# k2-fsa/Flow2GAN

Measured on AMD Instinct MI355X. Metric: audio-seconds/sec (train step, G+D fwd/bwd) mel_24k_base, higher is better.
Workload: dtype f32 (fp32-class products on the bf16 matrix pipe for the long reductions and the direct MRD convs: every fp32 operand as three bf16 pieces = 24 significand bits, the six v_mfma_f32_32x32x16_bf16 products with i + j <= 2 per fp32 product, fp32 accumulate, error <= 2^-23 per product; short reductions ; 1 GPU; mel_24k_base GAN stage-2 train step: D-step + G-step, each on its own batch (MPD+MRD+FM+multi-scale mel), fwd+bwd+grad all-reduce, no optimizer (metric is fwd/bwd); per_gpu_batch=64, gan=gan_multi_scale_mel_recon, parallelism=dp1, optimizer=none

## Files before the change

flow2gan_amd/_lib.py:

```python
from __future__ import annotations

import ctypes as C
import os

import torch

_HERE = os.path.dirname(os.path.abspath(__file__))
LIB_PATH = os.environ.get("F2G_LIB_PATH") or os.path.join(_HERE, "libflow2gan_hip.so")

c_float_p = C.c_void_p


class Operand(C.Structure):
    _fields_ = [
        ("base", C.c_void_p), ("rows", C.c_int32), ("cols", C.c_int32),
        ("P1", C.c_int32), ("P0", C.c_int32), ("seglen", C.c_int32),
        ("step1", C.c_int32), ("pad1", C.c_int32), ("L1", C.c_int32),
        ("step0", C.c_int32), ("pad0", C.c_int32), ("unit", C.c_int32), ("L0u", C.c_int32),
        ("seq_stride", C.c_int64), ("line_stride", C.c_int64),
        ("reflect", C.c_int32), ("split", C.c_int32),
        ("alpha", C.c_void_p), ("lrelu_src", C.c_void_p),
        ("lrelu_slope", C.c_float), ("unbounded", C.c_int32),
        ("rscale", C.c_void_p),
    ]
# ... 195 lines not shown
    "f2g_wave_gain": [_P, _L, _P, _L, _L, _I, _I, _I, _P, _P, _P],
    "f2g_sadam_stats": [_P, _P, _I, _P, _I],
    "f2g_sadam_prepare": [_P, C.POINTER(SadamGroup), _P, _P, _P, _P],
    "f2g_lrelu_bwd_colsum": [_P, _P, _P, _F, _P, _F, _I, _I, _L, _P],
    "f2g_lrelu_bwd_add": [_P, _P, _L, _I, _I, _I, _I, _L, _L, _L, _P, _L, _L, _L, _L, _F, _P],
    "f2g_zero_halo": [_P, _I, _I, _I, _I, _I],
    "f2g_sadam_update": [_P, _P, _I, _P],
    "f2g_mlp_pack": [_P, _P, _L, _P, _L, _I, _I],
    "f2g_fused_mlp": [C.POINTER(FusedMlpDesc)],
    "f2g_fused_block": [C.POINTER(DwnormFwd), C.POINTER(FusedMlpDesc)],
    "f2g_fused_block_multi": [C.POINTER(DwnormFwd), C.POINTER(FusedMlpDesc), C.c_int32],
    "f2g_istft_ola_multi": [C.POINTER(OlaMultiDesc), _P, _I, _I, _F, _I],
    "f2g_split_bf16x3": [_P, _P, _L, _I, _I],
    "f2g_split_f16x2": [_P, _P, _P, _L, _I, _I],
    "f2g_split_f16x2_cols": [_P, _P, _P, _P, _L, _I, _I],
    "f2g_split_f16x2_seq": [_P, _P, _P, _L, _I, _I],
    "f2g_multi": [C.POINTER(MultiDesc)],
}
EXPORTS = sorted(list(_SIGS) + ["f2g_version", "f2g_last_error", "f2g_gemm_last_path", "f2g_gemm_last_kernel",
                                 "f2g_fused_last_launch", "f2g_convnext_last_launch",
                                 "f2g_gemm_lean_ok", "f2g_gemm_wgrad_lean", "f2g_fused_mlp_ok",
                                 "f2g_dwnorm_bwd_workspace", "f2g_split_bf16x3_bytes", "f2g_gemm_x6_ok",
                                 "f2g_gemm_colsum_part_rows", "f2g_gemm_f16_ok", "f2g_set_option", "f2g_get_option",
                                 "f2g_dwconv_bwd_workspace", "f2g_sadam_chunk_elems"])


class F2GError(RuntimeError):
    pass


def _load():
    if not os.path.exists(LIB_PATH):
        raise ImportError(
            f"{LIB_PATH} is missing: build it with `python -c 'import __graft_entry__ as g; "
            "g.build()'` (or `make -C flow2gan_amd/csrc`). There is no CPU fallback.")
    lib = C.CDLL(LIB_PATH)
    for name, args in _SIGS.items():
        fn = getattr(lib, name)
        fn.argtypes = list(args) + [C.c_void_p]
        fn.restype = C.c_int
    for name in ("f2g_dwnorm_bwd_workspace", "f2g_dwconv_bwd_workspace"):
        fn = getattr(lib, name)
        fn.argtypes = [C.c_int32] * 4
        fn.restype = C.c_int64
    lib.f2g_gemm_lean_ok.argtypes = [C.POINTER(GemmDesc)]
    lib.f2g_gemm_lean_ok.restype = C.c_int
    lib.f2g_gemm_wgrad_lean.argtypes = [C.POINTER(GemmDesc)]
    lib.f2g_gemm_wgrad_lean.restype = C.c_int
    lib.f2g_split_bf16x3_bytes.argtypes = [C.c_int32, C.c_int32]
    lib.f2g_split_bf16x3_bytes.restype = C.c_int64
    lib.f2g_gemm_x6_ok.argtypes = [C.POINTER(GemmDesc)]
    lib.f2g_gemm_x6_ok.restype = C.c_int
    lib.f2g_gemm_f16_ok.argtypes = [C.POINTER(GemmDesc)]
    lib.f2g_gemm_f16_ok.restype = C.c_int
    lib.f2g_gemm_colsum_part_rows.argtypes = [C.POINTER(GemmDesc)]
    lib.f2g_gemm_colsum_part_rows.restype = C.c_int32
    lib.f2g_fused_mlp_ok.argtypes = [C.c_int32, C.c_int32]
    lib.f2g_fused_mlp_ok.restype = C.c_int
    lib.f2g_sadam_chunk_elems.argtypes = []
    lib.f2g_sadam_chunk_elems.restype = C.c_int32
    lib.f2g_set_option.argtypes = [C.c_char_p, C.c_int32]
    lib.f2g_set_option.restype = C.c_int
    lib.f2g_get_option.argtypes = [C.c_char_p, C.POINTER(C.c_int32)]
    lib.f2g_get_option.restype = C.c_int
    lib.f2g_version.restype = C.c_char_p
    lib.f2g_last_error.restype = C.c_char_p
    lib.f2g_gemm_last_kernel.argtypes = []
    lib.f2g_gemm_last_kernel.restype = C.c_char_p
    lib.f2g_fused_last_launch.argtypes = []
# ... 61 lines not shown
```

flow2gan_amd/csrc/capi.hip:

```cpp
#include <stdio.h>
#include <stdlib.h>
#include <string.h>
#include <strings.h>

#include <mutex>

#include "common.h"
#include "version_gen.h"

static char g_err[256] = "";

void f2g_set_error(const char* msg) {
  strncpy(g_err, msg ? msg : "", sizeof(g_err) - 1);
  g_err[sizeof(g_err) - 1] = 0;
}

int f2g_check_launch() {
  hipError_t e = hipGetLastError();
  if (e != hipSuccess) {
    f2g_set_error(hipGetErrorString(e));
    return F2G_ELAUNCH;
  }
  return F2G_OK;
}

extern "C" const char* f2g_version(void) { return "flow2gan_hip 0.4.0 src:" F2G_SRC_HASH " gfx950"; }
extern "C" const char* f2g_last_error(void) { return g_err; }

namespace {
struct Opt { const char* name; int value; };
Opt g_opts[F2G_OPT_COUNT] = {
    {"lean_tall", 1}, {"lean_wgrad", 1}, {"x6p", 1}, {"deterministic", 0}, {"streamk", 1}, {"mlp_rt", 0},
    {"mlp_split", 0}, {"multi_rt384", 4}, {"multi_rt512", 3}, {"streamk_min", 4}};
std::once_flag g_opts_once;

int opt_index(const char* name, size_t len) {
  for (int i = 0; i < F2G_OPT_COUNT; ++i)
    if (strlen(g_opts[i].name) == len && strncasecmp(g_opts[i].name, name, len) == 0) return i;
  return -1;
}

void opts_init() {
  const char* e = getenv("F2G_OPTS");
  while (e && *e) {
    const char* end = strchr(e, ',');
    const size_t len = end ? (size_t)(end - e) : strlen(e);
    const char* eq = (const char*)memchr(e, '=', len);
    if (eq) {
      const int i = opt_index(e, (size_t)(eq - e));
      if (i >= 0) g_opts[i].value = atoi(eq + 1);
    }
    e = end ? end + 1 : nullptr;
  }
  const char* det = getenv("F2G_DETERMINISTIC");
  if (det) g_opts[F2G_OPT_DETERMINISTIC].value = atoi(det) != 0;
}
// ... 26 lines not shown
```

flow2gan_amd/csrc/common.h:

```cpp
#pragma once
#include <hip/hip_runtime.h>
#include <stdint.h>

#include <type_traits>

#include "../../include/flow2gan_hip.h"

int f2g_check_launch();
void f2g_note_kernel(const char* name, int split, int path);
enum f2g_opt_id {
  F2G_OPT_LEAN_TALL,
  F2G_OPT_LEAN_WGRAD,
  F2G_OPT_X6P,
  F2G_OPT_DETERMINISTIC,
  F2G_OPT_STREAMK,
  F2G_OPT_MLP_RT,
  F2G_OPT_MLP_SPLIT,
  F2G_OPT_MULTI_RT384,
  F2G_OPT_MULTI_RT512,
  F2G_OPT_STREAMK_MIN,
  F2G_OPT_COUNT
};
int f2g_opt(int id);
int f2g_gemm_narrow(const f2g_gemm_desc& d, hipStream_t st);
void f2g_set_error(const char* msg);
int f2g_x6p_ok(const f2g_gemm_desc& d, int taps);
int f2g_launch_x6p(const f2g_gemm_desc& d, int taps, long long a_extent, hipStream_t st);
int f2g_leanw6t_ok(const f2g_gemm_desc& d, int split);
int f2g_launch_leanw6t(const f2g_gemm_desc& d, int split, hipStream_t st);
struct f2g_colsegs {
  float* out[3];
  int begin[3];
  int count[3];
};
int f2g_colsum_segments(const float* a, long long lda, int rows, int ncols,
                        const f2g_colsegs& segs, hipStream_t st);

#define F2G_WAVE 64

__device__ __forceinline__ float wave_sum(float v) {
#pragma unroll
  for (int o = 32; o > 0; o >>= 1) v += __shfl_xor(v, o);
  return v;
}

__device__ __forceinline__ float wave_max(float v) {
#pragma unroll
  for (int o = 32; o > 0; o >>= 1) v = fmaxf(v, __shfl_xor(v, o));
  return v;
}

typedef float f2g_f32x2 __attribute__((ext_vector_type(2)));
// ... 27 lines not shown
```

flow2gan_amd/csrc/gemm.hip:

```cpp
#include <hip/hip_runtime.h>
#include <stddef.h>
#include <stdint.h>
#include <stdio.h>
#include <string.h>

#include "gemm_common.h"

namespace {

int g_last_path = 0;
const char* g_last_kernel = "";
int g_last_split = 1;

struct RowCtx {
  long long base;
  int l1b, e0;
};

__device__ __forceinline__ RowCtx decode_row(const f2g_operand& S, int r) {
  RowCtx rc;
  int s, p1, p0;
  if (S.P0 == 1 && S.P1 == 1) {
    s = r; p1 = 0; p0 = 0;
  } else {
// ... 737 lines not shown
  hipLaunchKernelGGL(split_bf16_kernel, dim3((unsigned)blocks), dim3(256), 0, (hipStream_t)stream,
                     reinterpret_cast<uint4*>(dst), reinterpret_cast<const float4*>(src), n4);
  return f2g_check_launch();
}

extern "C" int f2g_gemm(const f2g_gemm_desc* dp, f2g_stream_t stream) {
  if (!dp || !dp->A.base || !dp->B.base || !dp->E.C) return F2G_EINVAL;
  f2g_note_kernel("", 1, g_last_path);
  const f2g_gemm_desc& d = *dp;
  hipStream_t st = (hipStream_t)stream;
  int split = d.split_k > 0 ? d.split_k : 1;
  if (d.E.colsum_part_ld > 0 && f2g_gemm_colsum_part_rows(dp) == 0) {
    f2g_set_error("f2g_gemm: E.colsum_part_ld needs a launch with the wide epilogue "
                  "(f2g_gemm_colsum_part_rows(d) == 0 for this descriptor)");
    return F2G_EINVAL;
  }
  if (d.precision == 4) return f2g_gemm_h3(d, st);
  if ((d.A.split >= 5 && d.A.split <= 8) || (d.B.split >= 5 && d.B.split <= 8)) {
    f2g_set_error("f2g_gemm: f2g_split_f16x2 / _cols / _seq images (split = 5 / 6 / 7) and maps scaled inside the "
                  "kernel (split = 8) belong to precision 4");
    return F2G_EINVAL;
  }
  if (d.precision == 3 && d.form == 2) {
    if (d.A.split || d.B.split || d.A.rows != d.B.rows || !f2g_leanw_ok(d) || d.E.x3_out ||
        (split > 1 && !d.E.atomic)) {
      f2g_set_error("f2g_gemm precision 3, form 2: fp32 operands the K-major weight-gradient kernel reads");
      return F2G_EINVAL;
    }
    return f2g_launch_leanw(d, 6, split, st);
  }
  if (d.precision == 3) return f2g_gemm_x6(d, st);
  if (d.E.x3_out) {
    f2g_set_error("f2g_gemm: E.x3_out belongs to precision 3");
    return F2G_EINVAL;
  }
  {
    const int nr = f2g_gemm_narrow(d, st);
    if (nr != 0) return nr < 0 ? nr : F2G_OK;
    f2g_note_kernel("", 1, 0);
  }
  if (d.E.prelu_slope && (d.E.atomic || d.E.accumulate || d.E.P0o > 0 || d.form == 2)) return F2G_EINVAL;
  if (d.E.mask_src && (d.E.atomic || d.E.accumulate || d.form == 2)) return F2G_EINVAL;
  if (d.form == 0 || d.form == 1) {
    const bool f1 = d.form == 1;
    if (f1 ? d.A.cols != d.B.rows : d.A.cols != d.B.cols) return F2G_EINVAL;
    if (!host_plain(d.B)) return F2G_EINVAL;
// ... 64 lines not shown
```

flow2gan_amd/csrc/gemm_x6.hip:

```cpp
#include <stddef.h>
#include <stdint.h>

#include "gemm_common.h"
#include "x6_epilogue.h"

#define X6_MFMA_PRIO 1

#if F2G_X6LAB & 256
__device__ unsigned long long g_x6prof[8];
extern "C" int f2g_lab_x6prof(unsigned long long* out8) {
  unsigned long long z[8] = {0, 0, 0, 0, 0, 0, 0, 0};
  if (hipMemcpyFromSymbol(out8, HIP_SYMBOL(g_x6prof), sizeof(z)) != hipSuccess) return 1;
  return hipMemcpyToSymbol(HIP_SYMBOL(g_x6prof), z, sizeof(z)) != hipSuccess;
}
#endif

__global__ __launch_bounds__(256) void split3_img_kernel(__bf16* __restrict__ dst, const float* __restrict__ src,
                                                         long long ld, long long rows, int K) {
  const long long total = rows * (K / 4);
  for (long long i = (long long)blockIdx.x * blockDim.x + threadIdx.x; i < total;
       i += (long long)gridDim.x * blockDim.x) {
    const long long r = i / (K / 4);
    const int k4 = (int)(i - r * (K / 4)) * 4;
    const float4 v = *reinterpret_cast<const float4*>(src + r * ld + k4);
// ... 599 lines not shown
  if (d.E.x3_out) {
    const f2g_epilogue& E = d.E;
    if (E.prelu_out || (((uintptr_t)E.x3_out) & 15) || (((uintptr_t)E.C) & 15) || (N % 8)) return false;
    if (E.P0o > 0 ? ((E.seq_stride_o | E.row_stride_o | E.off_o) & 7) != 0 : (E.ldc & 7) != 0) return false;
  }
  return true;
}

static int x6_wide(const f2g_gemm_desc& d) {
  return x6e::wide_ok(d.E, d.B.rows) ? 1 : 0;
}

static bool x6f_ok(const f2g_gemm_desc& d) {
  if (d.A.split || (d.B.split != 0 && d.B.split != 3 && d.B.split != 4) || !x6_shape_ok(d)) return false;
  if (d.B.split == 4 && ((d.B.rows & 31) || d.B.rows <= 32 || d.B.P0 != 1 || d.B.P1 != 1)) return false;
  if (!al16(d.A.base) || !al16(d.B.base) || (d.A.seq_stride & 3) || (d.B.split == 0 && (d.B.seq_stride & 3))) return false;
  const long long ext = host_plain(d.A) ? (long long)d.A.rows * d.A.seq_stride : x6_a_extent(d.A);
  return ext * 4 < 0xe0000000ll && (long long)d.B.rows * (d.B.split ? d.B.cols * 6ll : d.B.seq_stride * 4) < 0xe0000000ll;
}

enum x6_kind {
  X6_NONE,
  X6_P,
  X6_IMG,
  X6_F,
  X6_G,
  X6_N
};
struct x6_pick {
  x6_kind kind;
  int arg;
};

static x6_pick x6_choose(const f2g_gemm_desc& d) {
  if (x6f_ok(d)) {
    if (d.B.rows <= 32 && d.B.split == 3 && !d.E.x3_out) return {X6_N, 0};
    if (d.B.split == 4) return {X6_G, 0};
    return {X6_F, d.B.split == 3 ? 1 : 0};
  }
  if (d.A.split != 3 || d.B.split != 3 || !x6_shape_ok(d)) return {X6_NONE, 0};
  for (int taps = 5; taps >= 2; taps -= 3)
    if (x6_tap_ok(d, taps) && f2g_x6p_ok(d, taps)) return {X6_P, taps};
  return {X6_IMG, 0};
}

static x6_rows x6_rows_of(const f2g_operand& A, int es) {
  x6_rows R;
  if (host_plain(A)) {
    const long long pitch = es == 6 ? A.cols : A.seq_stride;
    R.P0 = 1, R.seq6 = (unsigned)(pitch * es), R.step6 = 0, R.off6 = 0;
    R.bytes = (unsigned)((long long)A.rows * pitch * es);
  } else {
    R.P0 = A.P0, R.seq6 = (unsigned)(A.seq_stride * es);
    R.step6 = (unsigned)((long long)A.step0 * A.unit * es), R.off6 = (unsigned)(-(long long)A.pad0 * A.unit * es);
    R.bytes = (unsigned)(x6_a_extent(A) * es);
  }
  return R;
}

int f2g_gemm_x6(const f2g_gemm_desc& d, hipStream_t st) {
  const int M = d.A.rows, N = d.B.rows, K = d.A.cols;
  constexpr size_t smem = 2 * 128 * 208;
  const dim3 grid((M + 127) / 128, (N + 127) / 128);
  const x6_pick pick = x6_choose(d);
  switch (pick.kind) {
    case X6_NONE:
      f2g_set_error("f2g_gemm precision 3: form 0 over plain f2g_split_bf16x3 images (split = 3), K % 32 == 0");
      return F2G_EINVAL;
    case X6_P:
      return f2g_launch_x6p(d, pick.arg, x6_a_extent(d.A), st);
    case X6_IMG:
      dyn_lds_once<gemm_x6_kernel>((int)smem);
      f2g_note_kernel("x6", 1, 4);
      hipLaunchKernelGGL(gemm_x6_kernel, grid, dim3(256), smem, st, d, M, N, K, x6_rows_of(d.A, 6), x6_wide(d));
      break;
    case X6_N: {
      constexpr size_t smem_n = (128 + 32) * 208;
      f2g_note_kernel("x6n", 1, 5);
      hipLaunchKernelGGL(gemm_x6n_kernel, dim3((M + 127) / 128), dim3(256), smem_n, st, d, M, N, K, x6_rows_of(d.A, 4));
      break;
    }
    case X6_G: {
      constexpr size_t smem_g = 4 * x6e::ESZ > 128 * 208 ? 4 * x6e::ESZ : 128 * 208;
      f2g_note_kernel("x6g", 1, 4);
      hipLaunchKernelGGL(gemm_x6g_kernel, grid, dim3(256), smem_g, st, d, M, N, K, x6_rows_of(d.A, 4), x6_wide(d));
      break;
    }
    case X6_F:
      dyn_lds_once<gemm_x6f_kernel<false>, gemm_x6f_kernel<true>>((int)smem);
      f2g_note_kernel(pick.arg ? "x6f<wimg=1>" : "x6f<wimg=0>", 1, 4);
      hipLaunchKernelGGL(pick.arg ? gemm_x6f_kernel<true> : gemm_x6f_kernel<false>, grid, dim3(256), smem, st, d, M, N,
                         K, x6_rows_of(d.A, 4), x6_wide(d));
      break;
  }
  return f2g_check_launch();
}

extern "C" int f2g_gemm_x6_ok(const f2g_gemm_desc* d) {
  if (!d || !x6_shape_ok(*d)) return 0;
  return 1 | ((x6_tap_ok(*d, 5) || x6_tap_ok(*d, 2)) ? 2 : 0) | (x6f_ok(*d) ? 4 : 0);
}

extern "C" int32_t f2g_gemm_colsum_part_rows(const f2g_gemm_desc* dp) {
  if (!dp || (dp->precision != 3 && dp->precision != 4) || dp->form != 0) return 0;
  f2g_gemm_desc d = *dp;
  if (d.E.colsum_part_ld <= 0) d.E.colsum_part_ld = 4;
  if (d.precision == 4 && d.A.split == 8) return f2g_h3p3n_ok(d) ? 2 * ((d.A.rows + 127) / 128) : 0;
  if (d.precision == 4) return f2g_h3p_ok(d, nullptr) || f2g_h3p3_ok(d) ? 4 * ((d.A.rows + 255) / 256) : 0;
  if (!x6_wide(d)) return 0;
  const int M = d.A.rows;
  switch (x6_choose(d).kind) {
    case X6_NONE:
    case X6_N:
      return 0;
    case X6_P:
      return 4 * ((M + 255) / 256);
    default:
      return 2 * ((M + 127) / 128);
  }
}

extern "C" int64_t f2g_split_bf16x3_bytes(int32_t rows, int32_t K) { return (int64_t)rows * K * 6; }

extern "C" int f2g_split_bf16x3(void* dst, const float* src, int64_t ld, int32_t rows, int32_t K,
                                f2g_stream_t stream) {
  if (!dst || !src || rows < 0 || K < 32 || (K % 32) || ld < K || (ld & 3) || (((uintptr_t)src) & 15) ||
      (((uintptr_t)dst) & 15))
    return F2G_EINVAL;
  if (rows == 0) return F2G_OK;
  const long long total = (long long)rows * (K / 4);
  hipLaunchKernelGGL(split3_img_kernel, dim3(f2g_grid_for(total, 256)), dim3(256), 0, (hipStream_t)stream,
                     reinterpret_cast<__bf16*>(dst), src, (long long)ld, (long long)rows, K);
  return f2g_check_launch();
}
```

flow2gan_amd/csrc/gemm_x6p.hip:

```cpp
#include <stdlib.h>

#include "gemm_common.h"
#include "x6_epilogue.h"

namespace {

constexpr int PITCH = 208;
constexpr int LH = 160;
constexpr int OPERA = 2 * LH * PITCH;
constexpr int OPERB = 128 * PITCH;
using x6e::ESZ;

struct x6p_tap {
  int P0, HpIn, offpos, C32;
  unsigned bytes;
};

template <int TAPS>
__global__ __launch_bounds__(512, 1) void gemm_x6p_kernel(const f2g_gemm_desc d, int M, int N, int K,
                                                          const x6p_tap R) {
  extern __shared__ __attribute__((aligned(16))) unsigned char smem6[];
  constexpr int NJA = (LH * 12 + 255) / 256, NJB = 128 * 12 / 512;
  const int tid = threadIdx.x, lane = tid & 63, wave = tid >> 6;
  const int grp = wave >> 2, gt = tid & 255;
// ... 89 lines not shown
            fb[ks][p][i] = *reinterpret_cast<const bf16x8*>(rB + buf * OPERB + p * 64 + i * 32 * PITCH + ks * 32);
          }
      storeB(buf ^ 1);
      gloadB(slab_of(step + 2));
      lds_barrier();
      if (t == TAPS - 1 && cs + 1 < R.C32) {
        storeA();
        gloadA(cs + 2 < R.C32 ? cs + 2 : 0);
      }
      __builtin_amdgcn_s_setprio(1);
#pragma unroll
      for (int ks = 0; ks < 2; ++ks)
#pragma unroll
        for (int sdeg = 2; sdeg >= 0; --sdeg)
#pragma unroll
          for (int i = 0; i < 3; ++i) {
            const int j = sdeg - i;
            if (j < 0 || j > 2) continue;
#pragma unroll
            for (int mi = 0; mi < 2; ++mi)
#pragma unroll
              for (int ni = 0; ni < 2; ++ni)
                acc[mi][ni] = __builtin_amdgcn_mfma_f32_32x32x16_bf16(fa[ks][i][mi], fb[ks][j][ni], acc[mi][ni], 0, 0, 0);
          }
      __builtin_amdgcn_s_setprio(0);
      if (!(grp == 1 && step == nsteps - 1)) lds_barrier();
    }
  }
  x6e::wide_epilogue(d.E, acc, M, N, mg + wm * 64, n0 + wn * 64, lane, smem6 + wave * ESZ);
}



template <int TAPS>
__global__ __launch_bounds__(512, 1) void gemm_leanw6t_kernel(const f2g_gemm_desc d, int K, int kchunk,
                                                              long long xrows) {
  constexpr int XR = 32 + TAPS - 1;
  constexpr int GPL = 32 * 256, XPL = XR * 256;
  constexpr int BUFB = 3 * GPL + 3 * XPL;
  constexpr int NXQ = (XR * 32 + 511) / 512;
  extern __shared__ __attribute__((aligned(16))) unsigned char smw[];
  const int tid = threadIdx.x, lane = tid & 63, wave = tid >> 6;
  const int wm = wave & 1, wq = wave >> 1, li = lane & 31, h = lane >> 5;
  const int m0 = blockIdx.x * 128, c0 = blockIdx.y * 128;
  const int kbeg = blockIdx.z * kchunk;
  int kend = kbeg + kchunk;
// ... 253 lines not shown
  const int mode = f2g_opt(F2G_OPT_X6P);
  if (mode == 0 || (taps != 5 && taps != 2)) return 0;
  if (d.A.unit / 32 < 2) return 0;
  if (!x6e::wide_ok(d.E, d.B.rows)) return 0;
  const long long tiles = (long long)((d.A.rows + 255) / 256) * ((d.B.rows + 127) / 128);
  return (mode >= 2 || tiles >= 256) ? 1 : 0;
}

int f2g_launch_x6p(const f2g_gemm_desc& d, int taps, long long a_extent, hipStream_t st) {
  const int M = d.A.rows, N = d.B.rows, K = d.A.cols;
  constexpr size_t smem = (size_t)OPERA + 2 * OPERB;
  static_assert(8 * ESZ <= (int)smem, "epilogue patches fit under the main loop's buffers");
  dyn_lds_once<gemm_x6p_kernel<5>, gemm_x6p_kernel<2>>((int)smem);
  x6p_tap R;
  R.P0 = d.A.P0, R.HpIn = (int)(d.A.seq_stride / d.A.unit), R.offpos = -d.A.pad0, R.C32 = d.A.unit / 32;
  R.bytes = (unsigned)(a_extent * 6);
  dim3 grid((M + 255) / 256, (N + 127) / 128);
  f2g_note_kernel(taps == 5 ? "x6p<taps=5>" : "x6p<taps=2>", 1, 4);
  if (taps == 5) hipLaunchKernelGGL(gemm_x6p_kernel<5>, grid, dim3(512), smem, st, d, M, N, K, R);
  else hipLaunchKernelGGL(gemm_x6p_kernel<2>, grid, dim3(512), smem, st, d, M, N, K, R);
  return f2g_check_launch();
}

int f2g_leanw6t_ok(const f2g_gemm_desc& d, int split) {
  const f2g_operand& A = d.A;
  const f2g_operand& B = d.B;
  if (d.form != 2 || d.precision != 3 || !d.E.atomic || d.E.P0o > 0 || d.E.bias || d.E.res) return 0;
  const f2g_epilogue& E = d.E;
  if ((E.scale != 0.f && E.scale != 1.f) || E.colsum || E.colsum_alpha || E.lrelu_slope != 0.f || E.mask_src ||
      E.aux || E.prelu_slope || E.c_bf16 || E.x3_out || E.accumulate || A.lrelu_src || A.alpha || B.lrelu_src || B.alpha)
    return 0;
  if (B.P1 != 1 || B.P0 < 1 || (B.step0 != 1 && B.step0 != 3) || B.unit < 128 || (B.unit % 128) || !B.unbounded) return 0;
  if (B.cols != 5 * B.unit || B.seglen < B.cols || (B.seq_stride % B.unit) || (B.rows % B.P0)) return 0;
  if (A.cols % 128 || A.rows != B.rows || B.pad0 < 0 || B.pad0 > 8) return 0;
  if (B.step0 == 1 && B.seq_stride != (long long)B.P0 * B.unit) return 0;
  const long long xrows = (long long)(B.rows / B.P0) * (B.seq_stride / B.unit);
  if (xrows * B.unit * 4 >= 0x7ff00000ll || (long long)A.rows * A.seq_stride * 4 >= 0x7ff00000ll) return 0;
  return 1;
}

int f2g_launch_leanw6t(const f2g_gemm_desc& d, int split, hipStream_t st) {
  const int M = d.A.cols, K = d.A.rows, Cin = d.B.unit;
  constexpr int TAPS = 5;
  if (d.B.step0 == 3) {
    constexpr size_t smem3 = (size_t)2 * (3 * 16 * 256 + 3 * (15 * 3 + TAPS) * 256);
    dyn_lds_once<gemm_leanw6s_kernel<5, 3>>((int)smem3);
// ... 41 lines not shown
```

flow2gan_amd/ops.py:

```python
from __future__ import annotations

import ctypes as C
from typing import Optional

import torch

from . import _lib as L
from ._opts import opt
from ._lib import DwconvBwd, DwnormBwd, DwnormFwd, Epilogue, GemmDesc, Operand, call, ptr


def empty(*shape, device, dtype=torch.float32):
    return torch.empty(*shape, device=device, dtype=dtype)


def zeros(*shape, device):
    t = torch.empty(*shape, device=device, dtype=torch.float32)
    fill_(t, 0.0)
    return t


def fill_(t, v: float):
    if BATCH is not None and t.numel() > 0:
        import struct
# ... 430 lines not shown
        if X6F == 2 and 128 <= A.cols < X6_MIN_K and A.rows >= X6F_TALL_ROWS and Bm.rows == 32:
            in_kernel = True
        if X6F == 2 and X6_MIN_K <= A.cols < X6_NOPASS_K and A.P0 == 1 and A.P1 == 1 and not _is_const(A._keep[0]):
            in_kernel = True
        if form == 0 and A.split == 0 and Bm.split == 0 and A.rows >= X6_MIN_ROWS \
                and (A.cols >= X6_MIN_K or in_kernel) and not atomic \
                and split_k <= 1 and out.dtype == torch.float32 and _x3_window_ok(A):
            how = _ask_with_x3_out(d, out, out_offset, x3_out, prelu_out, lambda: L.lib.f2g_gemm_x6_ok(C.byref(d)))
            if how:
                if in_kernel and not (how & 4):
                    in_kernel = False
                    how = how if A.cols >= X6_MIN_K else 0
                if how:
                    if not in_kernel:
                        d.A, d.B = _x3_operand(A), _x3_operand(Bm)
                    elif Bm.P0 == 1 and Bm.P1 == 1 and _is_const(Bm._keep[0]):
                        d.B = _x3_operand(Bm, frag_major=X6G and Bm.rows % 32 == 0 and Bm.rows > 32)
                    d.precision = 3
            if d.precision != 3:
                d.E.x3_out = None
        if form == 2 and atomic and A.split == 0 and Bm.split == 0 and A.lrelu_src is None \
                and A.rows >= X6_MIN_K and L.lib.f2g_gemm_lean_ok(C.byref(d)):
            d.precision = 3
        if x3_out:
            if d.E.x3_out:
                out._f2g_x3 = out._f2g_x3_buf
            else:
                out._f2g_x3_bad = True
    if (GEMM_PRECISION == 1 and form in (0, 2)) or (GEMM_PRECISION == 2 and form == 0):
        ok = L.lib.f2g_gemm_lean_ok(C.byref(d))
        if GEMM_PRECISION == 2 and (ok & 2):
            d.A, d.B = _bf16_operand(A), _bf16_operand(Bm)
        elif ok:
            d.A, d.B = _split_operand(A), _split_operand(Bm)
    parts = None
    if COLSUM_PARTS and d.precision in (3, 4) and form == 0 and (colsum is not None or colsum_alpha is not None) \
            and A.rows >= COLSUM_PARTS_MIN_ROWS:
        nrows = L.lib.f2g_gemm_colsum_part_rows(C.byref(d))
        if nrows > 0:
            ncol = Bm.rows
            both = colsum is not None and colsum_alpha is not None
            parts = torch.empty(nrows, (2 if both else 1) * ncol, device=out.device, dtype=torch.float32)
            d.E.colsum_part_ld = parts.stride(0)
            if colsum_alpha is not None:
                d.E.colsum_alpha = ptr(parts)
            if colsum is not None:
# ... 1406 lines not shown
```

include/flow2gan_hip.h:

```cpp
#ifndef FLOW2GAN_HIP_H
#define FLOW2GAN_HIP_H

#include <stdint.h>

#ifdef __cplusplus
extern "C" {
#endif

typedef void* f2g_stream_t;

enum {
  F2G_OK = 0,
  F2G_EINVAL = -1,
  F2G_ELAUNCH = -2,
};

const char* f2g_version(void);
const char* f2g_last_error(void);

int f2g_set_option(const char* name, int32_t value);
int f2g_get_option(const char* name, int32_t* value);

typedef struct {
  const float* base;
// ... 35 lines not shown
  float* prelu_out;
  int64_t ld_prelu_out;
  const float* mask_src;
  const float* fm_ref;
  const float* fm_wdev;
  float mask_slope;
  float fm_w;
  void* x3_out;
  int64_t colsum_part_ld;
} f2g_epilogue;

typedef struct {
  f2g_operand A, B;
  f2g_epilogue E;
  int32_t form;
  int32_t split_k;
  int32_t precision;
  int32_t _pad3;
} f2g_gemm_desc;

int f2g_gemm(const f2g_gemm_desc* d, f2g_stream_t stream);
int f2g_gemm_wgrad_lean(const f2g_gemm_desc* d);
int f2g_gemm_lean_ok(const f2g_gemm_desc* d);
int f2g_split_bf16(float* dst, const float* src, int64_t n, f2g_stream_t stream);
int f2g_to_bf16(void* dst, const float* src, int64_t n, f2g_stream_t stream);
int64_t f2g_split_bf16x3_bytes(int32_t rows, int32_t K);
int f2g_split_bf16x3(void* dst, const float* src, int64_t ld, int32_t rows, int32_t K, f2g_stream_t stream);
int f2g_gemm_x6_ok(const f2g_gemm_desc* d);
int32_t f2g_gemm_colsum_part_rows(const f2g_gemm_desc* d);
int f2g_split_f16x2(float* dst, float* rscale, const float* src, int64_t ld, int32_t rows, int32_t K,
                    f2g_stream_t stream);
int f2g_gemm_f16_ok(const f2g_gemm_desc* d);
int f2g_split_f16x2_cols(float* dst, float* rscale, uint32_t* work, const float* src, int64_t ld, int32_t rows,
                         int32_t cols, f2g_stream_t stream);
int f2g_split_f16x2_seq(float* dst, float* rscale, const float* src, int64_t ld, int32_t nseq, int32_t seq_floats,
                        f2g_stream_t stream);

int f2g_gemm_last_path(void);
const char* f2g_gemm_last_kernel(void);

typedef struct {
  const float* x;
  int64_t ldx;
  float* z;
  int64_t ldz;
  int32_t B, F, C, K;
// ... 326 lines not shown
```

Baseline: 810.8 audio-s/s.

## Add specialized bf16x3 kernels for stride-3 five-tap conv forward and weight gradient

Adds two new MFMA kernels specialized for the stride-3, 5-tap conv pattern used in the MPD discriminator. The first, x6p3, is a forward kernel that stages each input plane once in LDS and reuses it across taps in an interleaved tap order. The second, leanw6n, is a weight-gradient kernel that splits fp32 into three bf16 planes while staging and reads them with transposed LDS loads, then accumulates taps atomically. Both come with new eligibility checks and option flags, and the Python dispatcher now routes matching weight-gradient GEMMs to leanw6n. The aim is to cut the im2col-style operand traffic and split passes for these convs, at the cost of more code paths and atomic-add nondeterminism.

Measured after the change: 816.6 audio-s/s, median of 6. No clear change (+0.7%).

```diff
diff --git a/flow2gan_amd/_lib.py b/flow2gan_amd/_lib.py
--- a/flow2gan_amd/_lib.py
+++ b/flow2gan_amd/_lib.py
@@ -241,7 +241,7 @@
                                  "f2g_gemm_lean_ok", "f2g_gemm_wgrad_lean", "f2g_fused_mlp_ok",
                                  "f2g_dwnorm_bwd_workspace", "f2g_split_bf16x3_bytes", "f2g_gemm_x6_ok",
                                  "f2g_gemm_colsum_part_rows", "f2g_gemm_f16_ok", "f2g_set_option", "f2g_get_option",
-                                 "f2g_dwconv_bwd_workspace", "f2g_sadam_chunk_elems"])
+                                 "f2g_dwconv_bwd_workspace", "f2g_sadam_chunk_elems", "f2g_leanw6n_ok"])
 
 
 class F2GError(RuntimeError):
@@ -264,6 +264,8 @@
         fn.restype = C.c_int64
     lib.f2g_gemm_lean_ok.argtypes = [C.POINTER(GemmDesc)]
     lib.f2g_gemm_lean_ok.restype = C.c_int
+    lib.f2g_leanw6n_ok.argtypes = [C.POINTER(GemmDesc)]
+    lib.f2g_leanw6n_ok.restype = C.c_int
     lib.f2g_gemm_wgrad_lean.argtypes = [C.POINTER(GemmDesc)]
     lib.f2g_gemm_wgrad_lean.restype = C.c_int
     lib.f2g_split_bf16x3_bytes.argtypes = [C.c_int32, C.c_int32]
diff --git a/flow2gan_amd/csrc/capi.hip b/flow2gan_amd/csrc/capi.hip
--- a/flow2gan_amd/csrc/capi.hip
+++ b/flow2gan_amd/csrc/capi.hip
@@ -31,7 +31,7 @@
 struct Opt { const char* name; int value; };
 Opt g_opts[F2G_OPT_COUNT] = {
     {"lean_tall", 1}, {"lean_wgrad", 1}, {"x6p", 1}, {"deterministic", 0}, {"streamk", 1}, {"mlp_rt", 0},
-    {"mlp_split", 0}, {"multi_rt384", 4}, {"multi_rt512", 3}, {"streamk_min", 4}};
+    {"mlp_split", 0}, {"multi_rt384", 4}, {"multi_rt512", 3}, {"streamk_min", 4}, {"leanw6n", 1}, {"x6p3", 1}};
 std::once_flag g_opts_once;
 
 int opt_index(const char* name, size_t len) {
diff --git a/flow2gan_amd/csrc/common.h b/flow2gan_amd/csrc/common.h
--- a/flow2gan_amd/csrc/common.h
+++ b/flow2gan_amd/csrc/common.h
@@ -19,6 +19,8 @@
   F2G_OPT_MULTI_RT384,
   F2G_OPT_MULTI_RT512,
   F2G_OPT_STREAMK_MIN,
+  F2G_OPT_LEANW6N,
+  F2G_OPT_X6P3,
   F2G_OPT_COUNT
 };
 int f2g_opt(int id);
@@ -26,8 +28,12 @@
 void f2g_set_error(const char* msg);
 int f2g_x6p_ok(const f2g_gemm_desc& d, int taps);
 int f2g_launch_x6p(const f2g_gemm_desc& d, int taps, long long a_extent, hipStream_t st);
+int f2g_x6p3_ok(const f2g_gemm_desc& d);
+int f2g_launch_x6p3(const f2g_gemm_desc& d, long long a_extent, hipStream_t st);
 int f2g_leanw6t_ok(const f2g_gemm_desc& d, int split);
 int f2g_launch_leanw6t(const f2g_gemm_desc& d, int split, hipStream_t st);
+int f2g_leanw6n_takes(const f2g_gemm_desc& d);
+int f2g_launch_leanw6n(const f2g_gemm_desc& d, hipStream_t st);
 struct f2g_colsegs {
   float* out[3];
   int begin[3];
diff --git a/flow2gan_amd/csrc/gemm.hip b/flow2gan_amd/csrc/gemm.hip
--- a/flow2gan_amd/csrc/gemm.hip
+++ b/flow2gan_amd/csrc/gemm.hip
@@ -783,6 +783,7 @@
     return F2G_EINVAL;
   }
   if (d.precision == 3 && d.form == 2) {
+    if (f2g_leanw6n_takes(d)) return f2g_launch_leanw6n(d, st);
     if (d.A.split || d.B.split || d.A.rows != d.B.rows || !f2g_leanw_ok(d) || d.E.x3_out ||
         (split > 1 && !d.E.atomic)) {
       f2g_set_error("f2g_gemm precision 3, form 2: fp32 operands the K-major weight-gradient kernel reads");
diff --git a/flow2gan_amd/csrc/gemm_leanw6n.hip b/flow2gan_amd/csrc/gemm_leanw6n.hip
--- /dev/null
+++ b/flow2gan_amd/csrc/gemm_leanw6n.hip
@@ -0,0 +1,207 @@
+#include <stddef.h>
+#include <stdint.h>
+
+#include "gemm_common.h"
+
+namespace {
+
+constexpr int R = 16;
+constexpr int NTHR = 256;
+constexpr int GP = 256, XP = 64;
+constexpr int GPL = R * GP;
+constexpr int XROWB = 32 * 4;
+
+struct leanw6n_args {
+  const float* g;
+  const float* x;
+  float* C;
+  long long ldc;
+  unsigned gbytes, xbytes, rowG;
+  int nseq, Hp, HpIn, pad, nslab, units, xrows;
+};
+
+__device__ __forceinline__ void leanw6n_put(unsigned char* p, int plane_bytes, const u32x4 v) {
+  u32x2 p0, p1, p2;
+  split3x4(v, p0, p1, p2);
+  *reinterpret_cast<u32x2*>(p) = p0;
+  *reinterpret_cast<u32x2*>(p + plane_bytes) = p1;
+  *reinterpret_cast<u32x2*>(p + 2 * plane_bytes) = p2;
+}
+
+template <int PITCH, int HALF>
+__device__ __forceinline__ bf16x8 tr_frag_p(const unsigned char* p) {
+  typedef s16x4 __attribute__((address_space(3))) * lds_p;
+  const s16x4 a = __builtin_amdgcn_ds_read_tr16_b64_v4i16((lds_p)(p));
+  const s16x4 b = __builtin_amdgcn_ds_read_tr16_b64_v4i16((lds_p)(p + HALF * PITCH));
+  const s16x8 v = __builtin_shufflevector(a, b, 0, 1, 2, 3, 4, 5, 6, 7);
+  return __builtin_bit_cast(bf16x8, v);
+}
+
+template <int TAPS, int STRIDE>
+__global__ __launch_bounds__(NTHR, 2) void gemm_leanw6n_kernel(const leanw6n_args a) {
+  constexpr int XR = (R - 1) * STRIDE + TAPS;
+  constexpr int XPL = XR * XP;
+  constexpr int XOFF = 3 * GPL;
+  constexpr int BUFB = 3 * GPL + 3 * XPL;
+  constexpr int NGQ = R * 32 / NTHR;
+  constexpr int NXQ = (XR * 8 + NTHR - 1) / NTHR;
+  static_assert(STRIDE % 2 == 1, "staged rows STRIDE apart must walk all four 64-byte bank groups");
+  static_assert(NGQ * NTHR == R * 32 && NXQ == 2 && XR > 32, "a gradient slab in whole chunks per thread");
+  extern __shared__ __attribute__((aligned(16))) unsigned char smn[];
+  const int tid = threadIdx.x, lane = tid & 63;
+  const int wave = __builtin_amdgcn_readfirstlane(tid >> 6);
+  const int li = lane & 31, h = lane >> 5;
+  const int u0 = (int)((long long)blockIdx.x * a.units / gridDim.x);
+  const int nt = (int)((long long)(blockIdx.x + 1) * a.units / gridDim.x) - u0;
+  if (nt <= 0) return;
+  __amdgpu_buffer_rsrc_t ra = __builtin_amdgcn_make_buffer_rsrc((void*)a.g, 0, a.gbytes, 0x00020000);
+  __amdgpu_buffer_rsrc_t rb = __builtin_amdgcn_make_buffer_rsrc((void*)a.x, 0, a.xbytes, 0x00020000);
+  const int cc = tid & 31, rg = tid >> 5, cx = tid & 7, rx = tid >> 3;
+  const unsigned colG = (unsigned)cc * 16u, colX = (unsigned)cx * 16u;
+  const int wofG = rg * GP + ((((cc >> 3) ^ (rg & 3))) << 6) + (cc & 7) * 8;
+  const int wofX = XOFF + rx * XP + cx * 8;
+  const bool xrow2 = tid < 8 * (XR - 32);
+  const int g4 = lane >> 4, i16 = lane & 15;
+  const int rrow = (g4 >> 1) * 8 + (i16 >> 2), within = (g4 & 1) * 32 + (i16 & 3) * 8;
+  const int rofA = rrow * GP + (((wave ^ (rrow & 3))) << 6) + within;
+  const int rofB = XOFF + STRIDE * rrow * XP + within;
+  f32x16 acc[TAPS];
+#pragma unroll
+  for (int t = 0; t < TAPS; ++t)
+#pragma unroll
+    for (int e = 0; e < 16; ++e) acc[t][e] = 0.f;
+
+  struct slab {
+    u32x4 g[NGQ], x[NXQ];
+  };
+  auto gload = [&](int j, slab& s) {
+    const bool on = j < nt;
+    const int u = u0 + j, sq = u / a.nslab, p0 = (u - sq * a.nslab) * R;
+#pragma unroll
+    for (int q = 0; q < NGQ; ++q) {
+      const int p = p0 + rg + 8 * q;
+      s.g[q] = __builtin_amdgcn_raw_buffer_load_b128(
+          ra, (on && p < a.Hp) ? (unsigned)(sq * a.Hp + p) * a.rowG + colG : 0x80000000u, 0, 0);
+    }
+    const int xb = sq * a.HpIn + STRIDE * p0 - a.pad;
+#pragma unroll
+    for (int q = 0; q < NXQ; ++q) {
+      const int xr = xb + rx + 32 * q;
+      const bool ok = on && (q == 0 || xrow2) && xr >= 0 && xr < a.xrows;
+      s.x[q] = __builtin_amdgcn_raw_buffer_load_b128(rb, ok ? (unsigned)xr * XROWB + colX : 0x80000000u, 0, 0);
+    }
+  };
+  auto put = [&](unsigned char* buf, const slab& s) {
+#pragma unroll
+    for (int q = 0; q < NGQ; ++q) leanw6n_put(buf + wofG + q * 8 * GP, GPL, s.g[q]);
+#pragma unroll
+    for (int q = 0; q < NXQ; ++q)
+      if (q == 0 || xrow2) leanw6n_put(buf + wofX + q * 32 * XP, XPL, s.x[q]);
+  };
+
+  slab sa, sb;
+  gload(0, sa);
+  gload(1, sb);
+  put(smn, sa);
+  gload(2, sa);
+  lds_barrier();
+  auto step = [&](int j, slab& nxt) {
+    const unsigned char* cur = smn + (j & 1) * BUFB;
+    bf16x8 fa[3];
+#pragma unroll
+    for (int pc = 0; pc < 3; ++pc) fa[pc] = tr_frag_p<GP, 4>(cur + pc * GPL + rofA);
+    put(smn + ((j + 1) & 1) * BUFB, nxt);
+    gload(j + 3, nxt);
+    __builtin_amdgcn_sched_barrier(0);
+    bf16x8 fb[2][3];
+#pragma unroll
+    for (int pc = 0; pc < 3; ++pc) fb[0][pc] = tr_frag_p<XP, 4 * STRIDE>(cur + pc * XPL + rofB);
+#pragma unroll
+    for (int t = 0; t < TAPS; ++t) {
+      if (t + 1 < TAPS) {
+#pragma unroll
+        for (int pc = 0; pc < 3; ++pc)
+          fb[(t + 1) & 1][pc] = tr_frag_p<XP, 4 * STRIDE>(cur + pc * XPL + rofB + (t + 1) * XP);
+      }
+#pragma unroll
+      for (int sdeg = 2; sdeg >= 0; --sdeg)
+#pragma unroll
+        for (int i = 0; i < 3; ++i) {
+          const int jj = sdeg - i;
+          if (jj < 0 || jj > 2) continue;
+          acc[t] = __builtin_amdgcn_mfma_f32_32x32x16_bf16(fa[i], fb[t & 1][jj], acc[t], 0, 0, 0);
+        }
+      __builtin_amdgcn_sched_barrier(0);
+    }
+    lds_barrier();
+  };
+  int j = 0;
+  for (; j + 1 < nt; j += 2) {
+    step(j, sb);
+    step(j + 1, sa);
+  }
+  if (j < nt) step(j, sb);
+#pragma unroll
+  for (int e = 0; e < 16; ++e) {
+    const int row = wave * 32 + (e & 3) + 8 * (e >> 2) + 4 * h;
+    float* crow = a.C + (long long)row * a.ldc + li;
+#pragma unroll
+    for (int t = 0; t < TAPS; ++t) atomicAdd(crow + t * 32, acc[t][e]);
+  }
+}
+
+int leanw6n_blocks(long long units) {
+  long long blocks = units / (256 / R);
+  if (blocks > 2 * 256) blocks = 2 * 256;
+  return blocks < 1 ? 1 : (int)blocks;
+}
+
+}
+
+int f2g_leanw6n_takes(const f2g_gemm_desc& d) {
+  const f2g_operand& A = d.A;
+  const f2g_operand& B = d.B;
+  const f2g_epilogue& E = d.E;
+  if (f2g_opt(F2G_OPT_LEANW6N) == 0) return 0;
+  if (d.form != 2 || !A.base || !B.base || !E.C) return 0;
+  if (A.split || B.split || A.rscale || B.rscale) return 0;
+  if (!E.atomic || E.P0o > 0 || E.bias || E.res) return 0;
+  if ((E.scale != 0.f && E.scale != 1.f) || E.colsum || E.colsum_alpha || E.colsum_part_ld > 0 ||
+      E.lrelu_slope != 0.f || E.mask_src || E.aux || E.prelu_slope || E.c_bf16 || E.x3_out || E.accumulate ||
+      A.lrelu_src || A.alpha || B.lrelu_src || B.alpha)
+    return 0;
+  if (!host_plain(A) || A.rows < 1 || A.cols != 128 || A.rows != B.rows || !al16(A.base) || (A.seq_stride & 3) ||
+      A.seq_stride < A.cols)
+    return 0;
+  if (B.P1 != 1 || B.L1 != 1 || B.P0 < 1 || B.step0 != 3 || B.unit != 32 || !B.unbounded || B.reflect ||
+      !al16(B.base))
+    return 0;
+  if (B.cols != 5 * B.unit || B.seglen < B.cols || (B.rows % B.P0) || B.pad0 < 0 || B.pad0 > 8) return 0;
+  if (B.seq_stride < B.unit || (B.seq_stride % B.unit) || E.ldc < B.cols) return 0;
+  const long long HpIn = B.seq_stride / B.unit;
+  if (3ll * (B.P0 - 1) + 5 - B.pad0 > HpIn + B.pad0) return 0;
+  const long long xrows = (long long)(B.rows / B.P0) * HpIn;
+  if (xrows * B.unit * 4 >= 0x7ff00000ll || (long long)A.rows * A.seq_stride * 4 >= 0x7ff00000ll) return 0;
+  return 1;
+}
+
+extern "C" int f2g_leanw6n_ok(const f2g_gemm_desc* dp) { return dp ? f2g_leanw6n_takes(*dp) : 0; }
+
+int f2g_launch_leanw6n(const f2g_gemm_desc& d, hipStream_t st) {
+  constexpr int TAPS = 5, STRIDE = 3;
+  constexpr size_t smem = (size_t)2 * (3 * GPL + 3 * ((R - 1) * STRIDE + TAPS) * XP);
+  leanw6n_args a;
+  a.g = d.A.base, a.x = d.B.base, a.C = d.E.C;
+  a.ldc = d.E.ldc;
+  a.nseq = d.A.rows / d.B.P0, a.Hp = d.B.P0, a.HpIn = (int)(d.B.seq_stride / d.B.unit), a.pad = d.B.pad0;
+  a.nslab = (a.Hp + R - 1) / R;
+  a.xrows = a.nseq * a.HpIn;
+  a.rowG = (unsigned)(d.A.seq_stride * 4);
+  a.gbytes = (unsigned)((long long)d.A.rows * d.A.seq_stride * 4);
+  a.xbytes = (unsigned)a.xrows * XROWB;
+  const long long units = (long long)a.nseq * a.nslab;
+  a.units = (int)units;
+  f2g_note_kernel("leanw6n<step=3>", 1, 4);
+  hipLaunchKernelGGL((gemm_leanw6n_kernel<5, 3>), dim3(leanw6n_blocks(units)), dim3(NTHR), smem, st, a);
+  return f2g_check_launch();
+}
diff --git a/flow2gan_amd/csrc/gemm_x6.hip b/flow2gan_amd/csrc/gemm_x6.hip
--- a/flow2gan_amd/csrc/gemm_x6.hip
+++ b/flow2gan_amd/csrc/gemm_x6.hip
@@ -645,6 +645,7 @@
 enum x6_kind {
   X6_NONE,
   X6_P,
+  X6_P3,
   X6_IMG,
   X6_F,
   X6_G,
@@ -664,6 +665,7 @@
   if (d.A.split != 3 || d.B.split != 3 || !x6_shape_ok(d)) return {X6_NONE, 0};
   for (int taps = 5; taps >= 2; taps -= 3)
     if (x6_tap_ok(d, taps) && f2g_x6p_ok(d, taps)) return {X6_P, taps};
+  if (x6_tap3_ok(d, 160) && f2g_x6p3_ok(d)) return {X6_P3, 0};
   return {X6_IMG, 0};
 }
 
@@ -692,6 +694,8 @@
       return F2G_EINVAL;
     case X6_P:
       return f2g_launch_x6p(d, pick.arg, x6_a_extent(d.A), st);
+    case X6_P3:
+      return f2g_launch_x6p3(d, x6_a_extent(d.A), st);
     case X6_IMG:
       dyn_lds_once<gemm_x6_kernel>((int)smem);
       f2g_note_kernel("x6", 1, 4);
@@ -721,7 +725,7 @@
 
 extern "C" int f2g_gemm_x6_ok(const f2g_gemm_desc* d) {
   if (!d || !x6_shape_ok(*d)) return 0;
-  return 1 | ((x6_tap_ok(*d, 5) || x6_tap_ok(*d, 2)) ? 2 : 0) | (x6f_ok(*d) ? 4 : 0);
+  return 1 | ((x6_tap_ok(*d, 5) || x6_tap_ok(*d, 2)) ? 2 : 0) | (x6f_ok(*d) ? 4 : 0) | (x6_tap3_ok(*d, 160) ? 8 : 0);
 }
 
 extern "C" int32_t f2g_gemm_colsum_part_rows(const f2g_gemm_desc* dp) {
@@ -737,6 +741,7 @@
     case X6_N:
       return 0;
     case X6_P:
+    case X6_P3:
       return 4 * ((M + 255) / 256);
     default:
       return 2 * ((M + 127) / 128);
diff --git a/flow2gan_amd/csrc/gemm_x6p.hip b/flow2gan_amd/csrc/gemm_x6p.hip
--- a/flow2gan_amd/csrc/gemm_x6p.hip
+++ b/flow2gan_amd/csrc/gemm_x6p.hip
@@ -135,6 +135,158 @@
 #pragma unroll
               for (int ni = 0; ni < 2; ++ni)
                 acc[mi][ni] = __builtin_amdgcn_mfma_f32_32x32x16_bf16(fa[ks][i][mi], fb[ks][j][ni], acc[mi][ni], 0, 0, 0);
+          }
+      __builtin_amdgcn_s_setprio(0);
+      if (!(grp == 1 && step == nsteps - 1)) lds_barrier();
+    }
+  }
+  x6e::wide_epilogue(d.E, acc, M, N, mg + wm * 64, n0 + wn * 64, lane, smem6 + wave * ESZ);
+}
+
+
+struct x6p3_tap {
+  int P0, HpIn, offpos, C32;
+  unsigned bytes;
+};
+
+template <int TAPS, int STRIDE>
+__global__ __launch_bounds__(512, 1) void gemm_x6p3_kernel(const f2g_gemm_desc d, int M, int N, int K,
+                                                           const x6p3_tap R) {
+  static_assert(TAPS == 5 && STRIDE == 3, "the tap order and the plane schedule below are those of (5, 3)");
+  extern __shared__ __attribute__((aligned(16))) unsigned char smem6[];
+  constexpr int NJA = (LH * 12 + 255) / 256, NJB = 128 * 12 / 512;
+  constexpr int ORDER[TAPS] = {0, 3, 1, 4, 2};
+  const int tid = threadIdx.x, lane = tid & 63, wave = tid >> 6;
+  const int grp = wave >> 2, gt = tid & 255;
+  const int wm = (wave >> 1) & 1, wn = wave & 1, li = lane & 31, h = lane >> 5;
+  int m0, n0;
+  tile_of_block(256, 128, m0, n0);
+  const int mg = m0 + 128 * grp;
+  f32x16 acc[2][2];
+#pragma unroll
+  for (int i = 0; i < 2; ++i)
+#pragma unroll
+    for (int j = 0; j < 2; ++j)
+#pragma unroll
+      for (int e = 0; e < 16; ++e) acc[i][j][e] = 0.f;
+  const int sq0 = mg / R.P0, rl0 = mg - sq0 * R.P0;
+  auto entry_of = [&](int r) {
+    const int sq = r / R.P0;
+    return (sq - sq0) * (R.P0 + 1) + (r - sq * R.P0) - rl0;
+  };
+  const int elast = mg < M ? entry_of(mg + 127 < M ? mg + 127 : M - 1) : -2;
+  const unsigned rowbytesA = (unsigned)R.C32 * 192u;
+  const unsigned rowbytesW = (unsigned)(K / 32) * 192u;
+  __amdgpu_buffer_rsrc_t rsA = __builtin_amdgcn_make_buffer_rsrc((void*)d.A.base, 0, R.bytes, 0x00020000);
+  __amdgpu_buffer_rsrc_t rsW = __builtin_amdgcn_make_buffer_rsrc((void*)d.B.base, 0, (unsigned)N * rowbytesW, 0x00020000);
+  unsigned char* myA = smem6 + grp * (LH * PITCH);
+  constexpr int EPR = 256 / 12;
+  static_assert(NJA * EPR >= LH && (NJA - 1) * EPR < LH, "the rounds cover a plane");
+  unsigned voA[NJA], voW[NJB], ok2 = 0u;
+  int loW[NJB];
+  const int qa = gt / 12, ca = gt - qa * 12;
+  const int loA = qa * PITCH + ca * 16;
+  const bool lastA = qa + (NJA - 1) * EPR < LH;
+#pragma unroll
+  for (int j = 0; j < NJA; ++j) {
+    const int q = qa + EPR * j;
+    const int y = q + rl0, k = y / (R.P0 + 1), u = y - k * (R.P0 + 1);
+    voA[j] = (qa < EPR && q <= elast + 1)
+                 ? (unsigned)((sq0 + k) * R.HpIn + R.offpos + STRIDE * u + 2) * rowbytesA + ca * 16
+                 : 0xf0000000u;
+    if (q <= elast && u < R.P0) ok2 |= 1u << j;
+  }
+#pragma unroll
+  for (int j = 0; j < NJB; ++j) {
+    const int id = tid + 512 * j, row = id / 12, c = id - row * 12;
+    voW[j] = (unsigned)(n0 + row) * rowbytesW + c * 16;
+    loW[j] = OPERA + row * PITCH + c * 16;
+  }
+  u32x4 xa[NJA], xw[NJB];
+  auto gloadA = [&](int cls, int cs) {
+    const unsigned move = cls == 0 ? 0u - 2u * rowbytesA : rowbytesA;
+#pragma unroll
+    for (int j = 0; j < NJA; ++j) {
+      voA[j] += move;
+      xa[j] = __builtin_amdgcn_raw_buffer_load_b128(
+          rsA, (cls != 2 || ((ok2 >> j) & 1u)) ? voA[j] : 0xf0000000u, cs * 192, 0);
+    }
+  };
+  auto gloadB = [&](int slab) {
+#pragma unroll
+    for (int j = 0; j < NJB; ++j) xw[j] = __builtin_amdgcn_raw_buffer_load_b128(rsW, voW[j], slab * 192, 0);
+  };
+  auto storeA = [&]() {
+    if (qa < EPR) {
+#pragma unroll
+      for (int j = 0; j < NJA; ++j)
+        if (j + 1 < NJA || lastA) *reinterpret_cast<u32x4*>(myA + loA + j * EPR * PITCH) = xa[j];
+    }
+  };
+  auto storeB = [&](int buf) {
+#pragma unroll
+    for (int j = 0; j < NJB; ++j) *reinterpret_cast<u32x4*>(smem6 + buf * OPERB + loW[j]) = xw[j];
+  };
+  const unsigned char* rA[2];
+#pragma unroll
+  for (int i = 0; i < 2; ++i) {
+    const int r = mg + wm * 64 + i * 32 + li;
+    rA[i] = myA + (r < M ? entry_of(r) : 0) * PITCH + h * 16;
+  }
+  const unsigned char* rB = smem6 + OPERA + (wn * 64 + li) * PITCH + h * 16;
+  const int nsteps = R.C32 * TAPS;
+  auto slab_of = [&](int s) {
+    if (s >= nsteps) s = 0;
+    const int c2 = s / TAPS, i2 = s - c2 * TAPS;
+    const int t2 = i2 == 0 ? 0 : (i2 == 1 ? 3 : (i2 == 2 ? 1 : (i2 == 3 ? 4 : 2)));
+    return t2 * R.C32 + c2;
+  };
+  gloadA(0, 0);
+  gloadB(slab_of(0));
+  storeA();
+  storeB(0);
+  gloadA(1, 0);
+  gloadB(slab_of(1));
+  lds_barrier();
+  if (grp == 1) lds_barrier();
+  int step = 0;
+  for (int cs = 0; cs < R.C32; ++cs) {
+#pragma unroll
+    for (int i = 0; i < TAPS; ++i, ++step) {
+      const int t = ORDER[i], buf = step & 1;
+      bf16x8 fa[2][3][2], fb[2][3][2];
+#pragma unroll
+      for (int ks = 0; ks < 2; ++ks)
+#pragma unroll
+        for (int p = 0; p < 3; ++p)
+#pragma unroll
+          for (int s = 0; s < 2; ++s) {
+            fa[ks][p][s] = *reinterpret_cast<const bf16x8*>(rA[s] + (t / STRIDE) * PITCH + p * 64 + ks * 32);
+            fb[ks][p][s] = *reinterpret_cast<const bf16x8*>(rB + buf * OPERB + p * 64 + s * 32 * PITCH + ks * 32);
+          }
+      storeB(buf ^ 1);
+      gloadB(slab_of(step + 2));
+      lds_barrier();
+      if (i == 1 || i == 3 || i == 4) {
+        const int nxt = i == 1 ? 1 : (i == 3 ? 2 : 0);
+        if (nxt != 0 || cs + 1 < R.C32) storeA();
+        const int req = nxt == 2 ? 0 : nxt + 1, rcs = nxt == 0 ? cs + 1 : (nxt == 2 ? cs + 1 : cs);
+        gloadA(req, rcs < R.C32 ? rcs : 0);
+      }
+      __builtin_amdgcn_s_setprio(1);
+#pragma unroll
+      for (int ks = 0; ks < 2; ++ks)
+#pragma unroll
+        for (int sdeg = 2; sdeg >= 0; --sdeg)
+#pragma unroll
+          for (int ii = 0; ii < 3; ++ii) {
+            const int jj = sdeg - ii;
+            if (jj < 0 || jj > 2) continue;
+#pragma unroll
+            for (int mi = 0; mi < 2; ++mi)
+#pragma unroll
+              for (int ni = 0; ni < 2; ++ni)
+                acc[mi][ni] = __builtin_amdgcn_mfma_f32_32x32x16_bf16(fa[ks][ii][mi], fb[ks][jj][ni], acc[mi][ni], 0, 0, 0);
           }
       __builtin_amdgcn_s_setprio(0);
       if (!(grp == 1 && step == nsteps - 1)) lds_barrier();
@@ -434,6 +586,29 @@
   return f2g_check_launch();
 }
 
+int f2g_x6p3_ok(const f2g_gemm_desc& d) {
+  const int mode = f2g_opt(F2G_OPT_X6P);
+  if (mode == 0 || f2g_opt(F2G_OPT_X6P3) == 0) return 0;
+  if (!x6e::wide_ok(d.E, d.B.rows)) return 0;
+  if (mode >= 2) return 1;
+  const long long tiles = (long long)((d.A.rows + 255) / 256) * ((d.B.rows + 127) / 128);
+  const long long rounds = (tiles + 255) / 256;
+  return (tiles >= 256 && tiles * 100 >= rounds * 256 * 85) ? 1 : 0;
+}
+
+int f2g_launch_x6p3(const f2g_gemm_desc& d, long long a_extent, hipStream_t st) {
+  const int M = d.A.rows, N = d.B.rows, K = d.A.cols;
+  constexpr size_t smem = (size_t)OPERA + 2 * OPERB;
+  dyn_lds_once<gemm_x6p3_kernel<5, 3>>((int)smem);
+  x6p3_tap R;
+  R.P0 = d.A.P0, R.HpIn = (int)(d.A.seq_stride / d.A.unit), R.offpos = -d.A.pad0, R.C32 = d.A.unit / 32;
+  R.bytes = (unsigned)(a_extent * 6);
+  dim3 grid((M + 255) / 256, (N + 127) / 128);
+  f2g_note_kernel("x6p3<taps=5,step=3>", 1, 4);
+  hipLaunchKernelGGL((gemm_x6p3_kernel<5, 3>), grid, dim3(512), smem, st, d, M, N, K, R);
+  return f2g_check_launch();
+}
+
 int f2g_leanw6t_ok(const f2g_gemm_desc& d, int split) {
   const f2g_operand& A = d.A;
   const f2g_operand& B = d.B;
diff --git a/flow2gan_amd/ops.py b/flow2gan_amd/ops.py
--- a/flow2gan_amd/ops.py
+++ b/flow2gan_amd/ops.py
@@ -476,6 +476,9 @@
         if form == 2 and atomic and A.split == 0 and Bm.split == 0 and A.lrelu_src is None \
                 and A.rows >= X6_MIN_K and L.lib.f2g_gemm_lean_ok(C.byref(d)):
             d.precision = 3
+        elif form == 2 and atomic and A.split == 0 and Bm.split == 0 and A.lrelu_src is None \
+                and A.rows >= X6_MIN_K and L.lib.f2g_leanw6n_ok(C.byref(d)):
+            d.precision = 3
         if x3_out:
             if d.E.x3_out:
                 out._f2g_x3 = out._f2g_x3_buf
diff --git a/include/flow2gan_hip.h b/include/flow2gan_hip.h
--- a/include/flow2gan_hip.h
+++ b/include/flow2gan_hip.h
@@ -81,6 +81,7 @@
 int f2g_gemm(const f2g_gemm_desc* d, f2g_stream_t stream);
 int f2g_gemm_wgrad_lean(const f2g_gemm_desc* d);
 int f2g_gemm_lean_ok(const f2g_gemm_desc* d);
+int f2g_leanw6n_ok(const f2g_gemm_desc* d);
 int f2g_split_bf16(float* dst, const float* src, int64_t n, f2g_stream_t stream);
 int f2g_to_bf16(void* dst, const float* src, int64_t n, f2g_stream_t stream);
 int64_t f2g_split_bf16x3_bytes(int32_t rows, int32_t K);
```
